# WestlyPark/StyleRenderer

Measured on AMD Instinct MI355X. Metric: generator fwd+bwd images/sec at 256^2, higher is better.
Workload: dtype f32

## Files before the change

### stylerenderer_amd/csrc/conv_wino.h

```cpp
#pragma once
#include <hip/hip_runtime.h>
#include <stdint.h>

struct WinoParams {
    const float* in;
    const float* u;
    const float* iscale;
    const float* oscale;
    const float* obias;
    float* out;
    int B, C, N, H, W;
    int tiles_x, tiles_y, tiles_n;
    int nba;
    const float* nz;
    const float* nz_w;
    const float* abias;
    int64_t nz_bstride;
    float alpha, gain;
    int ks, kchunks;
    float* partial;
};

struct WinoNba {
    const float* nz;
    const float* nz_w;
    const float* abias;
    int64_t nz_bstride;
    float alpha, gain;
};

bool sr_wino_eligible(int64_t B, int64_t C, int64_t N, int64_t H, int64_t W, const void* in, const void* out);
int64_t sr_wino_scratch_floats(int64_t C, int64_t N);
int sr_wino_split(int64_t B, int64_t C, int64_t N, int64_t H, int64_t W);
int64_t sr_wino_partial_floats(int64_t B, int64_t C, int64_t N, int64_t H, int64_t W);
int sr_wino_conv3x3(float* out, const float* in, const float* wt, int64_t ldw, const float* iscale,
                    const float* oscale, const float* obias, int64_t B, int64_t C, int64_t N, int64_t H, int64_t W,
                    float* u_scratch, hipStream_t st, const WinoNba* nba = nullptr, bool u_ready = false);

bool sr_wgrad_wino_eligible(int64_t B, int64_t C, int64_t N, int64_t H, int64_t W, const void* x, const void* gy);
int64_t sr_wgrad_wino_scratch_floats(int64_t B, int64_t C, int64_t N, int64_t H, int64_t W);
int sr_wgrad_wino_3x3(float* dwt, const float* x, const float* gy, const float* xscale, const float* gscale,
                      int64_t B, int64_t C, int64_t N, int64_t H, int64_t W, float* scratch, hipStream_t st);
```

### stylerenderer_amd/csrc/conv_wino.hip

```cpp
#include <type_traits>
#include "common.h"
#include "conv_wino.h"
#include <cstdlib>

namespace {

typedef float f32x16 __attribute__((ext_vector_type(16)));
typedef const void __attribute__((address_space(1)))* gptr_t;
typedef void __attribute__((address_space(3)))* lptr_t;

__device__ __attribute__((aligned(16))) const float g_wino_zero[4] = {0.f, 0.f, 0.f, 0.f};

constexpr int TW = 16, TH = 4;
constexpr int NB = 64;
constexpr int EH = 2 * TH + 2;
constexpr int LEAD = 3;
constexpr int EWP = 40;
constexpr int PLANE = EH * EWP;

#ifdef WINO_TIMING
__device__ long long g_wino_stamps[8 * 16384];
#define WINO_STAMP(i) do { if (tid == 0) { g_wino_stamps[(blockIdx.x & 16383) * 8 + (i)] = wall_clock64(); } } while (0)
#else
#define WINO_STAMP(i)
#endif

template <int KC>
struct WG {
    static constexpr int CQ = KC / 4;
    static constexpr int PPS = CQ * 512;
    static constexpr int UV = 8 * PPS;
    static constexpr int U_INSTR = UV / 256;
    static constexpr int D_FLOATS = KC * PLANE;
    static constexpr int D_INSTR = (D_FLOATS / 4 + 63) / 64;
    static constexpr int D_BUF = D_INSTR * 256;
    static constexpr int D_PER_WAVE = (D_INSTR + 3) / 4;
    static constexpr int PAD = 4 * UV + 2 * D_BUF;
    static constexpr int STY = PAD + 3 * 256;
};

template <int KC>
__global__ __launch_bounds__(256) void k_conv_wino(const WinoParams p) {
#if __HIP_DEVICE_COMPILE__
    using G = WG<KC>;
    extern __shared__ __attribute__((aligned(16))) float smem[];
    float* const ubuf = smem;
    float* const vbuf = smem + 2 * G::UV;
    float* const dbuf = smem + 4 * G::UV + 1;
    float* const sty = smem + G::STY;

    const int nwg = gridDim.x;
    int bid = blockIdx.x;
    {
        const int q = nwg / SR_NUM_XCD, r = nwg % SR_NUM_XCD, xcd = bid % SR_NUM_XCD;
        bid = (xcd < r ? xcd * (q + 1) : r * (q + 1) + (xcd - r) * q) + bid / SR_NUM_XCD;
    }
    const int slice = bid % p.ks;
    bid /= p.ks;
    const int n_t = bid % p.tiles_n;
    bid /= p.tiles_n;
    const int tx_i = bid % p.tiles_x;
    bid /= p.tiles_x;
    const int ty_i = bid % p.tiles_y;
    const int b = bid / p.tiles_y;
    const int oy0 = ty_i * (2 * TH), ox0 = tx_i * (2 * TW), n0 = n_t * NB;

    const int tid = threadIdx.x, lane = tid & 63;
    const int wave = __builtin_amdgcn_readfirstlane(tid >> 6);
    const int half = lane >> 5, l31 = lane & 31;
    const int wn = wave & 1, wt = wave >> 1;
    const int nchunks = p.kchunks;
    const int k_lo = slice * p.kchunks;
    const int all_chunks = p.C / KC;
    WINO_STAMP(0);
#ifdef WINO_TIMING
    const long long wino_c0 = clock64();
    if (tid == 0) {
        g_wino_stamps[(blockIdx.x & 16383) * 8 + 6] = __builtin_amdgcn_s_getreg((31 << 11) | 4);
        g_wino_stamps[(blockIdx.x & 16383) * 8 + 7] = __builtin_amdgcn_s_getreg((31 << 11) | 20);
    }
#endif

    int d_off[G::D_PER_WAVE];
#pragma unroll
    for (int i = 0; i < G::D_PER_WAVE; ++i) {
        const int j = wave + 4 * i;
        const int f = (j * 64 + lane) * 4;
        int off = 0x7FFFFFF0;
        if (j < G::D_INSTR && f < G::D_FLOATS) {
            const int c = f / PLANE, q = f % PLANE;
            const int r = q / EWP, cola = q % EWP;
            const int gy = oy0 - 1 + r, gx = ox0 - 4 + cola;
            if (gy >= 0 && gy < p.H && gx >= 0 && gx + 3 < p.W) off = ((c * p.H + gy) * p.W + gx) * 4;
        }
        d_off[i] = off;
    }
    const int chunk_in_bytes = KC * p.H * p.W * 4;
    const __amdgpu_buffer_rsrc_t r_in = __builtin_amdgcn_make_buffer_rsrc(
        const_cast<float*>(p.in + ((int64_t)b * p.C + (int64_t)k_lo * KC) * p.H * p.W), 0, nchunks * chunk_in_bytes,
        0x00020000);
    const __amdgpu_buffer_rsrc_t r_u = __builtin_amdgcn_make_buffer_rsrc(
        const_cast<float*>(p.u + ((int64_t)n_t * all_chunks + k_lo) * G::UV), 0, nchunks * G::UV * 4, 0x00020000);
    const int u_voff = lane * 16;

    auto dma_d1 = [&](int k, int buf, int i) {
        const int j = wave + 4 * i;
        float* dst = j < G::D_INSTR ? dbuf + buf * G::D_BUF + j * 256 : smem + G::PAD + (wave - 1) * 256;
        __builtin_amdgcn_raw_ptr_buffer_load_lds(r_in, (lptr_t)dst, 16, d_off[i], k * chunk_in_bytes, 0, 0);
    };
    auto dma_u1 = [&](int k, int buf, int i) {
        const int j = wave + 4 * i;
        __builtin_amdgcn_raw_ptr_buffer_load_lds(r_u, (lptr_t)(ubuf + buf * G::UV + j * 256), 16, u_voff,
                                                 (k * G::UV + j * 256) * 4, 0, 0);
    };
    auto dma_d = [&](int k, int buf) {
#pragma unroll
        for (int i = 0; i < G::D_PER_WAVE; ++i) dma_d1(k, buf, i);
    };
    auto dma_u = [&](int k, int buf) {
#pragma unroll
        for (int i = 0; i < G::U_INSTR / 4; ++i) dma_u1(k, buf, i);
    };

    static_assert(KC == 8, "two channel quads per chunk");
    const int t_cq = wave & 1, t_h = wave >> 1;
    const int t_ca = 4 * t_cq + t_h;
    const int t_rd = t_ca * PLANE + (2 * (lane >> 4)) * EWP + LEAD + 2 * (lane & 15);
    const int t_wr = t_cq * 512 + t_h * 128 + lane * 2;

    typedef float f2 __attribute__((ext_vector_type(2)));
    auto ld2 = [](const float* q) { return *reinterpret_cast<const f2*>(q); };
    auto st2 = [](float* q, f2 v) { *reinterpret_cast<f2*>(q) = v; };
    auto pk_add = [](f2 x, f2 y) { f2 r; asm("v_pk_add_f32 %0, %1, %2" : "=v"(r) : "v"(x), "v"(y)); return r; };
    auto pk_sub = [](f2 x, f2 y) {
        f2 r;
        asm("v_pk_add_f32 %0, %1, %2 neg_lo:[0,1] neg_hi:[0,1]" : "=v"(r) : "v"(x), "v"(y));
        return r;
    };
    auto pk_mul_s = [](f2 x, f2 sv, int ch) {
        f2 r;
        if (ch == 0) asm("v_pk_mul_f32 %0, %1, %2 op_sel:[0,0] op_sel_hi:[1,0]" : "=v"(r) : "v"(x), "v"(sv));
        else asm("v_pk_mul_f32 %0, %1, %2 op_sel:[0,1] op_sel_hi:[1,1]" : "=v"(r) : "v"(x), "v"(sv));
        return r;
    };
    auto pk_fms_s = [](f2 x, f2 sv, f2 y, int ch) {
        f2 r;
        if (ch == 0)
            asm("v_pk_fma_f32 %0, %1, %2, %3 op_sel:[0,0,0] op_sel_hi:[1,0,1] neg_lo:[0,0,1] neg_hi:[0,0,1]"
                : "=v"(r) : "v"(x), "v"(sv), "v"(y));
        else
            asm("v_pk_fma_f32 %0, %1, %2, %3 op_sel:[0,1,0] op_sel_hi:[1,1,1] neg_lo:[0,0,1] neg_hi:[0,0,1]"
                : "=v"(r) : "v"(x), "v"(sv), "v"(y));
        return r;
    };
    auto pk_fnma_s = [](f2 x, f2 sv, f2 y, int ch) {
        f2 r;
        if (ch == 0)
            asm("v_pk_fma_f32 %0, %1, %2, %3 op_sel:[0,0,0] op_sel_hi:[1,0,1] neg_lo:[1,0,0] neg_hi:[1,0,0]"
                : "=v"(r) : "v"(x), "v"(sv), "v"(y));
        else
            asm("v_pk_fma_f32 %0, %1, %2, %3 op_sel:[0,1,0] op_sel_hi:[1,1,1] neg_lo:[1,0,0] neg_hi:[1,0,0]"
                : "=v"(r) : "v"(x), "v"(sv), "v"(y));
        return r;
    };
    auto col01 = [](f2 tp, f2 tq) {
        f2 r;
        asm("v_pk_add_f32 %0, %1, %2 op_sel:[0,0] op_sel_hi:[1,0] neg_lo:[0,1] neg_hi:[0,0]" : "=v"(r) : "v"(tp), "v"(tq));
        return r;
    };
    auto col23 = [](f2 tp, f2 tq) {
        f2 r;
        asm("v_pk_add_f32 %0, %1, %2 op_sel:[0,1] op_sel_hi:[1,1] neg_lo:[0,1] neg_hi:[1,0]" : "=v"(r) : "v"(tq), "v"(tp));
        return r;
    };
    struct XF {
        f2 P[2][4], Q[2][4];
        f2 sp[2][2], sq[2][2];
        f2 tp[2][4], tq[2][4];
        f2 o01[2][4], o23[2][4];
    };
    auto xf_read = [&](XF& x, const float* d0, int r) {
#pragma unroll
        for (int ch = 0; ch < 2; ++ch) {
            x.P[ch][r] = ld2(d0 + ch * 2 * PLANE + r * EWP);
            x.Q[ch][r] = ld2(d0 + ch * 2 * PLANE + r * EWP + 2);
        }
    };
    auto xf_step = [&](XF& x, int step, f2 sv) {
#pragma unroll
        for (int ch = 0; ch < 2; ++ch) {
            if (step == 0) {
                x.sp[ch][0] = pk_mul_s(x.P[ch][1], sv, ch);
                x.sp[ch][1] = pk_mul_s(x.P[ch][2], sv, ch);
                x.sq[ch][0] = pk_mul_s(x.Q[ch][1], sv, ch);
                x.sq[ch][1] = pk_mul_s(x.Q[ch][2], sv, ch);
                x.tp[ch][0] = pk_fms_s(x.P[ch][0], sv, x.sp[ch][1], ch);
                x.tq[ch][0] = pk_fms_s(x.Q[ch][0], sv, x.sq[ch][1], ch);
            } else if (step == 1) {
                x.tp[ch][1] = pk_add(x.sp[ch][0], x.sp[ch][1]);
                x.tq[ch][1] = pk_add(x.sq[ch][0], x.sq[ch][1]);
                x.tp[ch][2] = pk_sub(x.sp[ch][1], x.sp[ch][0]);
                x.tq[ch][2] = pk_sub(x.sq[ch][1], x.sq[ch][0]);
                x.tp[ch][3] = pk_fnma_s(x.P[ch][3], sv, x.sp[ch][0], ch);
                x.tq[ch][3] = pk_fnma_s(x.Q[ch][3], sv, x.sq[ch][0], ch);
            } else {
#pragma unroll
                for (int q = 2 * (step - 2); q < 2 * (step - 2) + 2; ++q) {
                    x.o01[ch][q] = col01(x.tp[ch][q], x.tq[ch][q]);
                    x.o23[ch][q] = col23(x.tp[ch][q], x.tq[ch][q]);
                }
            }
        }
    };
    auto xf_write = [&](const XF& x, float* vout, int q) {
#pragma unroll
        for (int ch = 0; ch < 2; ++ch) {
            st2(vout + (2 * q) * G::PPS + ch * 256, x.o01[ch][q]);
            st2(vout + (2 * q + 1) * G::PPS + ch * 256, x.o23[ch][q]);
        }
    };
    auto transform = [&](int k, int dsel, int vsel) {
        const float* d0 = dbuf + dsel * G::D_BUF + t_rd;
        float* v = vbuf + vsel * G::UV + t_wr;
        f2 sv;
        sv.x = sty[k * KC + t_ca];
        sv.y = sty[k * KC + t_ca + 2];
        XF x;
#pragma unroll
        for (int r = 0; r < 4; ++r) xf_read(x, d0, r);
#pragma unroll
        for (int st = 0; st < 4; ++st) xf_step(x, st, sv);
#pragma unroll
        for (int q = 0; q < 4; ++q) xf_write(x, v, q);
    };

    f32x16 acc[16];
#pragma unroll
    for (int pos = 0; pos < 16; ++pos)
#pragma unroll
        for (int r = 0; r < 16; ++r) acc[pos][r] = 0.0f;

    const int a_off = (half * 64 + wn * 32 + l31) * 2;
    const int b_off = (half * 64 + wt * 32 + l31) * 2;

    dma_d(0, 0);
    dma_u(0, 0);
    if (nchunks > 1) dma_d(1, 1);
    for (int c = tid; c < nchunks * KC; c += 256)
        sty[c] = p.iscale ? p.iscale[(int64_t)b * p.C + k_lo * KC + c] : 1.0f;
    __builtin_amdgcn_s_waitcnt(0x0F70);
    __syncthreads();
    WINO_STAMP(1);
    transform(0, 0, 0);
    WINO_STAMP(2);

    static_assert(KC == 8, "the slot schedule below is written for two channel quads per chunk");
    f2 au[2][2][8], bv[2][2][8];
    auto mfma_step = [&](int cq, int m) {
        const int e = m >> 4, pos = m & 15, pp = pos >> 1;
        if (pos & 1) acc[pos] = __builtin_amdgcn_mfma_f32_32x32x2f32(au[cq][e][pp].y, bv[cq][e][pp].y, acc[pos], 0, 0, 0);
        else acc[pos] = __builtin_amdgcn_mfma_f32_32x32x2f32(au[cq][e][pp].x, bv[cq][e][pp].x, acc[pos], 0, 0, 0);
    };
    auto body = [&](int k, auto first_tag) {
        constexpr bool FIRST = decltype(first_tag)::value;
        __builtin_amdgcn_s_waitcnt(0x0F70);
        __syncthreads();
        const int kd = min(k + 2, nchunks - 1), ku = min(k + 1, nchunks - 1);
        const float* ub = ubuf + (k & 1) * G::UV + a_off;
        const float* vb_ = vbuf + (k & 1) * G::UV + b_off;
        const int kn = (k + 1 < nchunks) ? k + 1 : k;
        const float* d0 = dbuf + ((k + 1) & 1) * G::D_BUF + t_rd;
        float* vout = vbuf + ((k + 1) & 1) * G::UV + t_wr;
        f2 sab;
        sab.x = sty[kn * KC + t_ca];
        sab.y = sty[kn * KC + t_ca + 2];
        XF x;
        auto load_ops = [&](int cq, int pp) {
#pragma unroll
            for (int e = 0; e < 2; ++e) {
                au[cq][e][pp] = ld2(ub + pp * G::PPS + cq * 512 + e * 256);
                bv[cq][e][pp] = ld2(vb_ + pp * G::PPS + cq * 512 + e * 256);
            }
        };
#ifndef WINO_RD
#define WINO_RD "0123"
#define WINO_ST "4567"
#define WINO_WR "CDEF"
#define WINO_L0 "4567"
#define WINO_L1 "89AB"
#define WINO_DD "45"
#define WINO_DU "89AB"
#endif
        constexpr char RD[] = WINO_RD, ST[] = WINO_ST, WR[] = WINO_WR, L0[] = WINO_L0, L1[] = WINO_L1, DD[] = WINO_DD,
                       DU[] = WINO_DU;
        static_assert(sizeof(RD) == 5 && sizeof(ST) == 5 && sizeof(WR) == 5 && sizeof(L0) == 5 && sizeof(L1) == 5 &&
                      sizeof(DD) == 3 && sizeof(DU) == 5, "schedule strings");
        static_assert(G::D_PER_WAVE == 4 && G::U_INSTR / 4 == 8, "4 halo + 8 weight DMA instructions per wave");
#pragma unroll
        for (int s = 0; s < 16; ++s) {
            const int cq = (s < 8) ? 1 : 0, j = s & 7;
            const char d = s < 10 ? '0' + s : 'A' + (s - 10);
            if (!(FIRST && s < 8)) {
#pragma unroll
                for (int u = 0; u < 4; ++u) mfma_step(cq, 4 * j + u);
            }
#pragma unroll
            for (int i = 0; i < 4; ++i) {
                if (L0[i] == d) { load_ops(0, 2 * i); load_ops(0, 2 * i + 1); }
                if (L1[i] == d) { load_ops(1, 2 * i); load_ops(1, 2 * i + 1); }
            }
#ifndef WINO_NO_DMA
#pragma unroll
            for (int i = 0; i < 4; ++i) {
                if (i < 2 && DD[i] == d) { dma_d1(kd, k & 1, 2 * i); dma_d1(kd, k & 1, 2 * i + 1); }
                if (DU[i] == d) { dma_u1(ku, (k + 1) & 1, 2 * i); dma_u1(ku, (k + 1) & 1, 2 * i + 1); }
            }
#endif
#ifndef WINO_NO_XFORM
#pragma unroll
            for (int i = 0; i < 4; ++i) if (RD[i] == d) xf_read(x, d0, i);
#pragma unroll
            for (int i = 0; i < 4; ++i) if (ST[i] == d) xf_step(x, i, sab);
#pragma unroll
            for (int i = 0; i < 4; ++i) if (WR[i] == d) xf_write(x, vout, i);
#endif
            __builtin_amdgcn_sched_barrier(0);
        }
    };
    body(0, std::true_type{});
    for (int k = 1; k < nchunks; ++k) body(k, std::false_type{});
#pragma unroll
    for (int m = 0; m < 32; ++m) mfma_step(1, m);

    __builtin_amdgcn_s_waitcnt(0x0F70);
    WINO_STAMP(3);

    const int tile = wt * 32 + l31;
    const int oy = oy0 + 2 * (tile >> 4), ox = ox0 + 2 * (tile & 15);
    const int64_t plane = (int64_t)p.H * p.W;
    float nzv[2][2] = {{0.0f, 0.0f}, {0.0f, 0.0f}};
    if (p.nba && p.nz) {
#pragma clang fp contract(off)
        const float nw = p.nz_w[0];
        const float* nzp = p.nz + b * p.nz_bstride + (int64_t)oy * p.W + ox;
#pragma unroll
        for (int a = 0; a < 2; ++a) {
            nzv[a][0] = nw * nzp[a * p.W];
            nzv[a][1] = nw * nzp[a * p.W + 1];
        }
    }
#pragma unroll
    for (int r = 0; r < 16; ++r) {
        const int n = n0 + wn * 32 + (r & 3) + 8 * (r >> 2) + 4 * half;
        float s[2][4];
#pragma unroll
        for (int j = 0; j < 4; ++j) {
            const float m0 = acc[j][r], m1 = acc[4 + j][r], m2 = acc[8 + j][r], m3 = acc[12 + j][r];
            s[0][j] = (m0 + m1) + m2;
            s[1][j] = (m1 - m2) - m3;
        }
        if (p.ks > 1) {
            float* o = p.partial + (((int64_t)slice * p.B + b) * p.N + n) * plane + (int64_t)oy * p.W + ox;
            *reinterpret_cast<float2*>(o) = make_float2((s[0][0] + s[0][1]) + s[0][2], (s[0][1] - s[0][2]) - s[0][3]);
            *reinterpret_cast<float2*>(o + p.W) = make_float2((s[1][0] + s[1][1]) + s[1][2], (s[1][1] - s[1][2]) - s[1][3]);
            continue;
        }
        const float os = p.oscale ? p.oscale[(int64_t)b * p.N + n] : 1.0f;
        const float ob = p.obias ? p.obias[n] : 0.0f;
        float* o = p.out + ((int64_t)b * p.N + n) * plane + (int64_t)oy * p.W + ox;
        const float ab = (p.nba && p.abias) ? p.abias[n] : 0.0f;
        float y[2][2];
#pragma unroll
        for (int a = 0; a < 2; ++a) {
            const float y0 = (s[a][0] + s[a][1]) + s[a][2];
            const float y1 = (s[a][1] - s[a][2]) - s[a][3];
            float v0 = y0 * os + ob, v1 = y1 * os + ob;
            if (p.nba) {
#pragma clang fp contract(off)
                v0 = v0 + nzv[a][0];
                v1 = v1 + nzv[a][1];
                v0 = v0 + ab;
                v1 = v1 + ab;
                v0 = ((v0 > 0.0f) ? v0 : v0 * p.alpha) * p.gain;
                v1 = ((v1 > 0.0f) ? v1 : v1 * p.alpha) * p.gain;
            }
            y[a][0] = v0;
            y[a][1] = v1;
        }
        *reinterpret_cast<float2*>(o) = make_float2(y[0][0], y[0][1]);
        *reinterpret_cast<float2*>(o + p.W) = make_float2(y[1][0], y[1][1]);
    }
    WINO_STAMP(4);
#ifdef WINO_TIMING
    if (tid == 0) g_wino_stamps[(blockIdx.x & 16383) * 8 + 5] = clock64() - wino_c0;
#endif
#endif
}

__global__ __launch_bounds__(256) void k_wino_reduce(const WinoParams p) {
    const int64_t plane = (int64_t)p.H * p.W, total4 = (int64_t)p.B * p.N * plane / 4;
    const int64_t slab4 = total4;
    for (int64_t i = (int64_t)blockIdx.x * 256 + threadIdx.x; i < total4; i += (int64_t)gridDim.x * 256) {
        const float4* src = reinterpret_cast<const float4*>(p.partial) + i;
        float4 a = src[0];
        for (int s = 1; s < p.ks; ++s) {
            const float4 q = src[s * slab4];
            a.x += q.x; a.y += q.y; a.z += q.z; a.w += q.w;
        }
        const int64_t row = (i * 4) / plane;
        const int n = (int)(row % p.N), b = (int)(row / p.N);
        const int64_t pix = i * 4 - row * plane;
        const float os = p.oscale ? p.oscale[row] : 1.0f;
        const float ob = p.obias ? p.obias[n] : 0.0f;
        float v[4] = {a.x * os + ob, a.y * os + ob, a.z * os + ob, a.w * os + ob};
        if (p.nba) {
#pragma clang fp contract(off)
            const float ab = p.abias ? p.abias[n] : 0.0f;
            float nz[4] = {0.0f, 0.0f, 0.0f, 0.0f};
            if (p.nz) {
                const float nw = p.nz_w[0];
                const float4 q = *reinterpret_cast<const float4*>(p.nz + b * p.nz_bstride + pix);
                nz[0] = nw * q.x; nz[1] = nw * q.y; nz[2] = nw * q.z; nz[3] = nw * q.w;
            }
#pragma unroll
            for (int j = 0; j < 4; ++j) {
                float t = v[j] + nz[j];
                t = t + ab;
                v[j] = ((t > 0.0f) ? t : t * p.alpha) * p.gain;
            }
        }
        reinterpret_cast<float4*>(p.out)[i] = make_float4(v[0], v[1], v[2], v[3]);
    }
}

template <int KC>
__global__ __launch_bounds__(64) void k_wino_weights(float* __restrict__ u, const float* __restrict__ wt, int C,
                                                     int N, int ldw) {
    using G = WG<KC>;
    const int n = blockIdx.x * 64 + threadIdx.x, c = blockIdx.y;
    float g[3][3];
#pragma unroll
    for (int t = 0; t < 9; ++t) g[t / 3][t % 3] = wt[((int64_t)t * C + c) * ldw + n];
    float h[4][3];
#pragma unroll
    for (int j = 0; j < 3; ++j) {
        h[0][j] = g[0][j];
        h[1][j] = 0.5f * ((g[0][j] + g[2][j]) + g[1][j]);
        h[2][j] = 0.5f * ((g[0][j] + g[2][j]) - g[1][j]);
        h[3][j] = g[2][j];
    }
    const int cl = c % KC, cq = cl / 4, e = (cl % 4) / 2, hh = cl % 2;
    float* dst = u + ((int64_t)blockIdx.x * (C / KC) + c / KC) * G::UV + cq * 512 + e * 256 + hh * 128 + threadIdx.x * 2;
#pragma unroll
    for (int i = 0; i < 4; ++i) {
        *reinterpret_cast<float2*>(dst + (2 * i) * G::PPS) = make_float2(h[i][0], 0.5f * ((h[i][0] + h[i][2]) + h[i][1]));
        *reinterpret_cast<float2*>(dst + (2 * i + 1) * G::PPS) = make_float2(0.5f * ((h[i][0] + h[i][2]) - h[i][1]), h[i][2]);
    }
}

template <int KC>
int launch(const WinoParams& p, float* u, const float* wt, int ldw, hipStream_t st, bool u_ready) {
    using G = WG<KC>;
    const int lds = (G::STY + p.kchunks * KC) * 4;
    auto kern = k_conv_wino<KC>;
    static bool configured = false;
    if (!configured) {
        if (hipFuncSetAttribute(reinterpret_cast<const void*>(kern), hipFuncAttributeMaxDynamicSharedMemorySize,
                                160 * 1024) != hipSuccess) {
            (void)hipGetLastError();
            return SR_EINVAL;
        }
        configured = true;
    }
    if (!u_ready) hipLaunchKernelGGL(k_wino_weights<KC>, dim3(p.N / 64, p.C), dim3(64), 0, st, u, wt, p.C, p.N, ldw);
    const int64_t blocks = (int64_t)p.tiles_n * p.tiles_x * p.tiles_y * p.B * p.ks;
    hipLaunchKernelGGL(kern, dim3((unsigned)blocks), dim3(256), lds, st, p);
    if (p.ks > 1) {
        const int64_t total4 = (int64_t)p.B * p.N * p.H * p.W / 4;
        int64_t grid = (total4 + 255) / 256;
        if (grid > 8192) grid = 8192;
        hipLaunchKernelGGL(k_wino_reduce, dim3((unsigned)grid), dim3(256), 0, st, p);
    }
    return sr_launch_status();
}

}

#ifdef WINO_TIMING
extern "C" int sr_debug_wino_stamps(long long* host, int n) {
    return (int)hipMemcpyFromSymbol(host, HIP_SYMBOL(g_wino_stamps), (size_t)n * sizeof(long long));
}
#endif

bool sr_wino_eligible(int64_t B, int64_t C, int64_t N, int64_t H, int64_t W, const void* in, const void* out) {
    if (B <= 0 || C % 8 != 0 || N % 64 != 0 || H % 8 != 0 || W % 32 != 0) return false;
    if (C > 512 || B * ((W / 32) * (H / 8)) * (N / 64) > 0x7FFFFFFFLL) return false;
    if (C * H * W >= (1LL << 29) - 4 || 16 * C * 64 >= (1LL << 29)) return false;
    return ((reinterpret_cast<uintptr_t>(in) | reinterpret_cast<uintptr_t>(out)) & 15) == 0;
}

int64_t sr_wino_scratch_floats(int64_t C, int64_t N) { return 16 * C * N; }

int sr_wino_split(int64_t B, int64_t C, int64_t N, int64_t H, int64_t W) {
    const char* e = std::getenv("SR_WINO_SPLIT");
    if (e && e[0] == '0') return 1;
    const int64_t blocks = B * (W / (2 * TW)) * (H / (2 * TH)) * (N / NB), nchunks = C / 8;
    int ks = 1;
    while (blocks * ks < 192 && ks < 8 && nchunks % (2 * ks) == 0 && nchunks / (2 * ks) >= 8) ks *= 2;
    return ks;
}
int64_t sr_wino_partial_floats(int64_t B, int64_t C, int64_t N, int64_t H, int64_t W) {
    const int ks = sr_wino_split(B, C, N, H, W);
    return ks > 1 ? (int64_t)ks * B * N * H * W : 0;
}

int sr_wino_conv3x3(float* out, const float* in, const float* wt, int64_t ldw, const float* iscale,
                    const float* oscale, const float* obias, int64_t B, int64_t C, int64_t N, int64_t H, int64_t W,
                    float* u_scratch, hipStream_t st, const WinoNba* nba, bool u_ready) {
    WinoParams p;
    p.in = in; p.u = u_scratch; p.iscale = iscale; p.oscale = oscale; p.obias = obias; p.out = out;
    p.nba = nba ? 1 : 0;
    p.nz = nba ? nba->nz : nullptr; p.nz_w = nba ? nba->nz_w : nullptr; p.abias = nba ? nba->abias : nullptr;
    p.nz_bstride = nba ? nba->nz_bstride : 0; p.alpha = nba ? nba->alpha : 0.0f; p.gain = nba ? nba->gain : 1.0f;
    p.B = (int)B; p.C = (int)C; p.N = (int)N; p.H = (int)H; p.W = (int)W;
    p.tiles_x = (int)(W / (2 * TW)); p.tiles_y = (int)(H / (2 * TH)); p.tiles_n = (int)(N / NB);
    p.ks = sr_wino_split(B, C, N, H, W);
    p.kchunks = (int)(C / 8) / p.ks;
    p.partial = u_scratch + sr_wino_scratch_floats(C, N);
    return launch<8>(p, u_scratch, wt, (int)ldw, st, u_ready);
}
```

Baseline: 549.1.

## Make Winograd conv kernel persistent, overlapping next tile prologue with epilogue

Turns the Winograd 3x3 conv kernel into a persistent kernel: the grid is capped at the CU count and each workgroup loops over virtual tile IDs. Before running the current tile's epilogue it decodes the next tile, computes its DMA offsets, loads its style scales and issues the first halo/weight DMAs, so the next tile's loads overlap the output stores. The accumulator zeroing moves into the first MFMA step. Epilogue per-channel scales are loaded once per lane and broadcast with readlane. Risks include higher register pressure, worse load balance when tile counts are not a multiple of the grid, and buffer-parity bookkeeping across tiles.

```diff
diff --git a/stylerenderer_amd/csrc/conv_wino.h b/stylerenderer_amd/csrc/conv_wino.h
--- a/stylerenderer_amd/csrc/conv_wino.h
+++ b/stylerenderer_amd/csrc/conv_wino.h
@@ -19,6 +19,7 @@
     float alpha, gain;
     int ks, kchunks;
     float* partial;
+    int total;
 };
 
 struct WinoNba {
@@ -33,6 +34,7 @@
 int64_t sr_wino_scratch_floats(int64_t C, int64_t N);
 int sr_wino_split(int64_t B, int64_t C, int64_t N, int64_t H, int64_t W);
 int64_t sr_wino_partial_floats(int64_t B, int64_t C, int64_t N, int64_t H, int64_t W);
+int sr_wino_grid(int64_t tiles);
 int sr_wino_conv3x3(float* out, const float* in, const float* wt, int64_t ldw, const float* iscale,
                     const float* oscale, const float* obias, int64_t B, int64_t C, int64_t N, int64_t H, int64_t W,
                     float* u_scratch, hipStream_t st, const WinoNba* nba = nullptr, bool u_ready = false);
diff --git a/stylerenderer_amd/csrc/conv_wino.hip b/stylerenderer_amd/csrc/conv_wino.hip
--- a/stylerenderer_amd/csrc/conv_wino.hip
+++ b/stylerenderer_amd/csrc/conv_wino.hip
@@ -20,9 +20,11 @@
 
 #ifdef WINO_TIMING
 __device__ long long g_wino_stamps[8 * 16384];
-#define WINO_STAMP(i) do { if (tid == 0) { g_wino_stamps[(blockIdx.x & 16383) * 8 + (i)] = wall_clock64(); } } while (0)
+#define WINO_STAMP(i) do { if (tid == 0) { g_wino_stamps[(v & 16383) * 8 + (i)] = wall_clock64(); } } while (0)
+#define WINO_CLOCK() do { if (tid == 0) g_wino_stamps[(v & 16383) * 8 + 5] = clock64() - wino_c0; } while (0)
 #else
 #define WINO_STAMP(i)
+#define WINO_CLOCK()
 #endif
 
 template <int KC>
@@ -49,58 +51,53 @@
     float* const dbuf = smem + 4 * G::UV + 1;
     float* const sty = smem + G::STY;
 
-    const int nwg = gridDim.x;
-    int bid = blockIdx.x;
-    {
-        const int q = nwg / SR_NUM_XCD, r = nwg % SR_NUM_XCD, xcd = bid % SR_NUM_XCD;
-        bid = (xcd < r ? xcd * (q + 1) : r * (q + 1) + (xcd - r) * q) + bid / SR_NUM_XCD;
-    }
-    const int slice = bid % p.ks;
-    bid /= p.ks;
-    const int n_t = bid % p.tiles_n;
-    bid /= p.tiles_n;
-    const int tx_i = bid % p.tiles_x;
-    bid /= p.tiles_x;
-    const int ty_i = bid % p.tiles_y;
-    const int b = bid / p.tiles_y;
-    const int oy0 = ty_i * (2 * TH), ox0 = tx_i * (2 * TW), n0 = n_t * NB;
-
     const int tid = threadIdx.x, lane = tid & 63;
     const int wave = __builtin_amdgcn_readfirstlane(tid >> 6);
     const int half = lane >> 5, l31 = lane & 31;
     const int wn = wave & 1, wt = wave >> 1;
     const int nchunks = p.kchunks;
-    const int k_lo = slice * p.kchunks;
     const int all_chunks = p.C / KC;
-    WINO_STAMP(0);
-#ifdef WINO_TIMING
-    const long long wino_c0 = clock64();
-    if (tid == 0) {
-        g_wino_stamps[(blockIdx.x & 16383) * 8 + 6] = __builtin_amdgcn_s_getreg((31 << 11) | 4);
-        g_wino_stamps[(blockIdx.x & 16383) * 8 + 7] = __builtin_amdgcn_s_getreg((31 << 11) | 20);
-    }
-#endif
+    const int chunk_in_bytes = KC * p.H * p.W * 4;
+
+    struct Tile { int b, slice, n_t, oy0, ox0; };
+    const int xq = p.total / SR_NUM_XCD, xr = p.total % SR_NUM_XCD;
+    auto decode = [&](int vid) {
+        const int xcd = vid % SR_NUM_XCD;
+        int bid = (xcd < xr ? xcd * (xq + 1) : xr * (xq + 1) + (xcd - xr) * xq) + vid / SR_NUM_XCD;
+        Tile t;
+        t.slice = bid % p.ks;
+        bid /= p.ks;
+        t.n_t = bid % p.tiles_n;
+        bid /= p.tiles_n;
+        t.ox0 = (bid % p.tiles_x) * (2 * TW);
+        bid /= p.tiles_x;
+        t.oy0 = (bid % p.tiles_y) * (2 * TH);
+        t.b = bid / p.tiles_y;
+        return t;
+    };
 
     int d_off[G::D_PER_WAVE];
-#pragma unroll
-    for (int i = 0; i < G::D_PER_WAVE; ++i) {
-        const int j = wave + 4 * i;
-        const int f = (j * 64 + lane) * 4;
-        int off = 0x7FFFFFF0;
-        if (j < G::D_INSTR && f < G::D_FLOATS) {
+    __amdgpu_buffer_rsrc_t r_in, r_u;
+    auto aim = [&](const Tile& t) {
+        int ln = lane;
+        asm volatile("" : "+v"(ln));
+#pragma unroll
+        for (int i = 0; i < G::D_PER_WAVE; ++i) {
+            const int j = wave + 4 * i;
+            const int f = (j * 64 + ln) * 4;
             const int c = f / PLANE, q = f % PLANE;
             const int r = q / EWP, cola = q % EWP;
-            const int gy = oy0 - 1 + r, gx = ox0 - 4 + cola;
-            if (gy >= 0 && gy < p.H && gx >= 0 && gx + 3 < p.W) off = ((c * p.H + gy) * p.W + gx) * 4;
-        }
-        d_off[i] = off;
-    }
-    const int chunk_in_bytes = KC * p.H * p.W * 4;
-    const __amdgpu_buffer_rsrc_t r_in = __builtin_amdgcn_make_buffer_rsrc(
-        const_cast<float*>(p.in + ((int64_t)b * p.C + (int64_t)k_lo * KC) * p.H * p.W), 0, nchunks * chunk_in_bytes,
-        0x00020000);
-    const __amdgpu_buffer_rsrc_t r_u = __builtin_amdgcn_make_buffer_rsrc(
-        const_cast<float*>(p.u + ((int64_t)n_t * all_chunks + k_lo) * G::UV), 0, nchunks * G::UV * 4, 0x00020000);
+            const int gy = t.oy0 - 1 + r, gx = t.ox0 - 4 + cola;
+            const bool ok = (j < G::D_INSTR) & (f < G::D_FLOATS) & (gy >= 0) & (gy < p.H) & (gx >= 0) & (gx + 3 < p.W);
+            d_off[i] = ok ? ((c * p.H + gy) * p.W + gx) * 4 : 0x7FFFFFF0;
+        }
+        const int k_lo = t.slice * nchunks;
+        r_in = __builtin_amdgcn_make_buffer_rsrc(
+            const_cast<float*>(p.in + ((int64_t)t.b * p.C + (int64_t)k_lo * KC) * p.H * p.W), 0,
+            nchunks * chunk_in_bytes, 0x00020000);
+        r_u = __builtin_amdgcn_make_buffer_rsrc(
+            const_cast<float*>(p.u + ((int64_t)t.n_t * all_chunks + k_lo) * G::UV), 0, nchunks * G::UV * 4, 0x00020000);
+    };
     const int u_voff = lane * 16;
 
     auto dma_d1 = [&](int k, int buf, int i) {
@@ -235,53 +232,80 @@
     };
 
     f32x16 acc[16];
-#pragma unroll
-    for (int pos = 0; pos < 16; ++pos)
-#pragma unroll
-        for (int r = 0; r < 16; ++r) acc[pos][r] = 0.0f;
 
     const int a_off = (half * 64 + wn * 32 + l31) * 2;
     const int b_off = (half * 64 + wt * 32 + l31) * 2;
 
-    dma_d(0, 0);
-    dma_u(0, 0);
-    if (nchunks > 1) dma_d(1, 1);
-    for (int c = tid; c < nchunks * KC; c += 256)
-        sty[c] = p.iscale ? p.iscale[(int64_t)b * p.C + k_lo * KC + c] : 1.0f;
-    __builtin_amdgcn_s_waitcnt(0x0F70);
-    __syncthreads();
-    WINO_STAMP(1);
-    transform(0, 0, 0);
-    WINO_STAMP(2);
-
-    static_assert(KC == 8, "the slot schedule below is written for two channel quads per chunk");
-    f2 au[2][2][8], bv[2][2][8];
-    auto mfma_step = [&](int cq, int m) {
-        const int e = m >> 4, pos = m & 15, pp = pos >> 1;
-        if (pos & 1) acc[pos] = __builtin_amdgcn_mfma_f32_32x32x2f32(au[cq][e][pp].y, bv[cq][e][pp].y, acc[pos], 0, 0, 0);
-        else acc[pos] = __builtin_amdgcn_mfma_f32_32x32x2f32(au[cq][e][pp].x, bv[cq][e][pp].x, acc[pos], 0, 0, 0);
-    };
-    auto body = [&](int k, auto first_tag) {
-        constexpr bool FIRST = decltype(first_tag)::value;
-        __builtin_amdgcn_s_waitcnt(0x0F70);
-        __syncthreads();
-        const int kd = min(k + 2, nchunks - 1), ku = min(k + 1, nchunks - 1);
-        const float* ub = ubuf + (k & 1) * G::UV + a_off;
-        const float* vb_ = vbuf + (k & 1) * G::UV + b_off;
-        const int kn = (k + 1 < nchunks) ? k + 1 : k;
-        const float* d0 = dbuf + ((k + 1) & 1) * G::D_BUF + t_rd;
-        float* vout = vbuf + ((k + 1) & 1) * G::UV + t_wr;
-        f2 sab;
-        sab.x = sty[kn * KC + t_ca];
-        sab.y = sty[kn * KC + t_ca + 2];
-        XF x;
-        auto load_ops = [&](int cq, int pp) {
-#pragma unroll
-            for (int e = 0; e < 2; ++e) {
-                au[cq][e][pp] = ld2(ub + pp * G::PPS + cq * 512 + e * 256);
-                bv[cq][e][pp] = ld2(vb_ + pp * G::PPS + cq * 512 + e * 256);
-            }
+    static_assert(KC == 8, "style row: at most 512 channels per tile, see sr_wino_eligible");
+    float sreg[2];
+    auto style_load = [&](const Tile& t) {
+        int th = tid;
+        asm volatile("" : "+v"(th));
+#pragma unroll
+        for (int i = 0; i < 2; ++i) {
+            const int c = th + 256 * i;
+            sreg[i] = (p.iscale && c < nchunks * KC) ? p.iscale[(int64_t)t.b * p.C + t.slice * nchunks * KC + c] : 1.0f;
+        }
+    };
+    auto style_store = [&]() {
+        int th = tid;
+        asm volatile("" : "+v"(th));
+#pragma unroll
+        for (int i = 0; i < 2; ++i) {
+            const int c = th + 256 * i;
+            if (c < nchunks * KC) sty[c] = sreg[i];
+        }
+    };
+    auto issue_first = [&](int par) {
+        dma_d(0, par);
+        dma_u(0, par);
+        dma_d(min(1, nchunks - 1), par ^ 1);
+    };
+
+    int v = blockIdx.x, par = 0;
+    Tile cur = decode(v);
+#ifdef WINO_TIMING
+    const int wino_hw0 = __builtin_amdgcn_s_getreg((31 << 11) | 4), wino_hw1 = __builtin_amdgcn_s_getreg((31 << 11) | 20);
+#endif
+    aim(cur);
+    style_load(cur);
+    issue_first(0);
+    for (;;) {
+        static_assert(KC == 8, "the slot schedule below is written for two channel quads per chunk");
+        f2 au[2][2][8], bv[2][2][8];
+        auto mfma_step = [&](int cq, int m, bool start) {
+            const int e = m >> 4, pos = m & 15, pp = pos >> 1;
+            f32x16 c;
+            if (start) {
+#pragma unroll
+                for (int r = 0; r < 16; ++r) c[r] = 0.0f;
+            } else {
+                c = acc[pos];
+            }
+            if (pos & 1) acc[pos] = __builtin_amdgcn_mfma_f32_32x32x2f32(au[cq][e][pp].y, bv[cq][e][pp].y, c, 0, 0, 0);
+            else acc[pos] = __builtin_amdgcn_mfma_f32_32x32x2f32(au[cq][e][pp].x, bv[cq][e][pp].x, c, 0, 0, 0);
         };
+        auto body = [&](int k, int kb, auto first_tag) {
+            constexpr bool FIRST = decltype(first_tag)::value;
+            __builtin_amdgcn_s_waitcnt(0x0F70);
+            __syncthreads();
+            const int kd = min(k + 2, nchunks - 1), ku = min(k + 1, nchunks - 1);
+            const float* ub = ubuf + (kb & 1) * G::UV + a_off;
+            const float* vb_ = vbuf + (kb & 1) * G::UV + b_off;
+            const int kn = (k + 1 < nchunks) ? k + 1 : k;
+            const float* d0 = dbuf + ((kb + 1) & 1) * G::D_BUF + t_rd;
+            float* vout = vbuf + ((kb + 1) & 1) * G::UV + t_wr;
+            f2 sab;
+            sab.x = sty[kn * KC + t_ca];
+            sab.y = sty[kn * KC + t_ca + 2];
+            XF x;
+            auto load_ops = [&](int cq, int pp) {
+#pragma unroll
+                for (int e = 0; e < 2; ++e) {
+                    au[cq][e][pp] = ld2(ub + pp * G::PPS + cq * 512 + e * 256);
+                    bv[cq][e][pp] = ld2(vb_ + pp * G::PPS + cq * 512 + e * 256);
+                }
+            };
 #ifndef WINO_RD
 #define WINO_RD "0123"
 #define WINO_ST "4567"
@@ -291,109 +315,165 @@
 #define WINO_DD "45"
 #define WINO_DU "89AB"
 #endif
-        constexpr char RD[] = WINO_RD, ST[] = WINO_ST, WR[] = WINO_WR, L0[] = WINO_L0, L1[] = WINO_L1, DD[] = WINO_DD,
-                       DU[] = WINO_DU;
-        static_assert(sizeof(RD) == 5 && sizeof(ST) == 5 && sizeof(WR) == 5 && sizeof(L0) == 5 && sizeof(L1) == 5 &&
-                      sizeof(DD) == 3 && sizeof(DU) == 5, "schedule strings");
-        static_assert(G::D_PER_WAVE == 4 && G::U_INSTR / 4 == 8, "4 halo + 8 weight DMA instructions per wave");
-#pragma unroll
-        for (int s = 0; s < 16; ++s) {
-            const int cq = (s < 8) ? 1 : 0, j = s & 7;
-            const char d = s < 10 ? '0' + s : 'A' + (s - 10);
-            if (!(FIRST && s < 8)) {
-#pragma unroll
-                for (int u = 0; u < 4; ++u) mfma_step(cq, 4 * j + u);
-            }
-#pragma unroll
-            for (int i = 0; i < 4; ++i) {
-                if (L0[i] == d) { load_ops(0, 2 * i); load_ops(0, 2 * i + 1); }
-                if (L1[i] == d) { load_ops(1, 2 * i); load_ops(1, 2 * i + 1); }
-            }
+            constexpr char RD[] = WINO_RD, ST[] = WINO_ST, WR[] = WINO_WR, L0[] = WINO_L0, L1[] = WINO_L1, DD[] = WINO_DD,
+                           DU[] = WINO_DU;
+            static_assert(sizeof(RD) == 5 && sizeof(ST) == 5 && sizeof(WR) == 5 && sizeof(L0) == 5 && sizeof(L1) == 5 &&
+                          sizeof(DD) == 3 && sizeof(DU) == 5, "schedule strings");
+            static_assert(G::D_PER_WAVE == 4 && G::U_INSTR / 4 == 8, "4 halo + 8 weight DMA instructions per wave");
+#pragma unroll
+            for (int s = 0; s < 16; ++s) {
+                const int cq = (s < 8) ? 1 : 0, j = s & 7;
+                const char d = s < 10 ? '0' + s : 'A' + (s - 10);
+                if (!(FIRST && s < 8)) {
+#pragma unroll
+                    for (int u = 0; u < 4; ++u) mfma_step(cq, 4 * j + u, FIRST && 4 * j + u < 16);
+                }
+#pragma unroll
+                for (int i = 0; i < 4; ++i) {
+                    if (L0[i] == d) { load_ops(0, 2 * i); load_ops(0, 2 * i + 1); }
+                    if (L1[i] == d) { load_ops(1, 2 * i); load_ops(1, 2 * i + 1); }
+                }
 #ifndef WINO_NO_DMA
 #pragma unroll
-            for (int i = 0; i < 4; ++i) {
-                if (i < 2 && DD[i] == d) { dma_d1(kd, k & 1, 2 * i); dma_d1(kd, k & 1, 2 * i + 1); }
-                if (DU[i] == d) { dma_u1(ku, (k + 1) & 1, 2 * i); dma_u1(ku, (k + 1) & 1, 2 * i + 1); }
-            }
+                for (int i = 0; i < 4; ++i) {
+                    if (i < 2 && DD[i] == d) { dma_d1(kd, kb & 1, 2 * i); dma_d1(kd, kb & 1, 2 * i + 1); }
+                    if (DU[i] == d) { dma_u1(ku, (kb + 1) & 1, 2 * i); dma_u1(ku, (kb + 1) & 1, 2 * i + 1); }
+                }
 #endif
 #ifndef WINO_NO_XFORM
 #pragma unroll
-            for (int i = 0; i < 4; ++i) if (RD[i] == d) xf_read(x, d0, i);
-#pragma unroll
-            for (int i = 0; i < 4; ++i) if (ST[i] == d) xf_step(x, i, sab);
-#pragma unroll
-            for (int i = 0; i < 4; ++i) if (WR[i] == d) xf_write(x, vout, i);
-#endif
-            __builtin_amdgcn_sched_barrier(0);
-        }
-    };
-    body(0, std::true_type{});
-    for (int k = 1; k < nchunks; ++k) body(k, std::false_type{});
-#pragma unroll
-    for (int m = 0; m < 32; ++m) mfma_step(1, m);
-
+                for (int i = 0; i < 4; ++i) if (RD[i] == d) xf_read(x, d0, i);
+#pragma unroll
+                for (int i = 0; i < 4; ++i) if (ST[i] == d) xf_step(x, i, sab);
+#pragma unroll
+                for (int i = 0; i < 4; ++i) if (WR[i] == d) xf_write(x, vout, i);
+#endif
+                __builtin_amdgcn_sched_barrier(0);
+            }
+        };
+        WINO_STAMP(0);
+#ifdef WINO_TIMING
+        const long long wino_c0 = clock64();
+        if (tid == 0) {
+            g_wino_stamps[(v & 16383) * 8 + 6] = wino_hw0;
+            g_wino_stamps[(v & 16383) * 8 + 7] = wino_hw1;
+        }
+#endif
+        style_store();
+        __builtin_amdgcn_s_waitcnt(0x0F70);
+        __syncthreads();
+        WINO_STAMP(1);
+        transform(0, par, par);
+        WINO_STAMP(2);
+        body(0, par, std::true_type{});
+        for (int k = 1; k < nchunks; ++k) body(k, k + par, std::false_type{});
+        WINO_STAMP(3);
+
+        const int b = cur.b, n0 = cur.n_t * NB;
+        const int tile = wt * 32 + l31;
+        const int oy = cur.oy0 + 2 * (tile >> 4), ox = cur.ox0 + 2 * (tile & 15);
+        const int64_t plane = (int64_t)p.H * p.W;
+        const int nl = n0 + wn * 32 + 4 * half;
+        float e_os = 1.0f, e_ob = 0.0f, e_ab = 0.0f;
+        float nzv[2][2] = {{0.0f, 0.0f}, {0.0f, 0.0f}}, nzw = 0.0f;
+        if (p.ks == 1) {
+            const int nc = n0 + wn * 32 + l31;
+            if (p.oscale) e_os = p.oscale[(int64_t)b * p.N + nc];
+            if (p.obias) e_ob = p.obias[nc];
+            if (p.nba && p.abias) e_ab = p.abias[nc];
+            if (p.nba && p.nz) {
+                nzw = p.nz_w[0];
+                const float* nzp = p.nz + b * p.nz_bstride + (int64_t)oy * p.W + ox;
+#pragma unroll
+                for (int a = 0; a < 2; ++a) {
+                    nzv[a][0] = nzp[a * p.W];
+                    nzv[a][1] = nzp[a * p.W + 1];
+                }
+            }
+        }
+        __builtin_amdgcn_sched_barrier(0);
+#pragma unroll
+        for (int m = 0; m < 32; ++m) mfma_step(1, m, false);
+        __builtin_amdgcn_sched_barrier(0);
+
+        auto epilogue = [&]() {
+            if (p.nba && p.nz) {
+#pragma clang fp contract(off)
+#pragma unroll
+                for (int a = 0; a < 2; ++a) {
+                    nzv[a][0] = nzw * nzv[a][0];
+                    nzv[a][1] = nzw * nzv[a][1];
+                }
+            }
+#pragma unroll
+            for (int r = 0; r < 16; ++r) {
+                const int n = nl + (r & 3) + 8 * (r >> 2);
+                float s[2][4];
+#pragma unroll
+                for (int j = 0; j < 4; ++j) {
+                    const float m0 = acc[j][r], m1 = acc[4 + j][r], m2 = acc[8 + j][r], m3 = acc[12 + j][r];
+                    s[0][j] = (m0 + m1) + m2;
+                    s[1][j] = (m1 - m2) - m3;
+                }
+                if (p.ks > 1) {
+                    float* o = p.partial + (((int64_t)cur.slice * p.B + b) * p.N + n) * plane + (int64_t)oy * p.W + ox;
+                    *reinterpret_cast<float2*>(o) = make_float2((s[0][0] + s[0][1]) + s[0][2], (s[0][1] - s[0][2]) - s[0][3]);
+                    *reinterpret_cast<float2*>(o + p.W) = make_float2((s[1][0] + s[1][1]) + s[1][2], (s[1][1] - s[1][2]) - s[1][3]);
+                    continue;
+                }
+                const int c0 = (r & 3) + 8 * (r >> 2);
+                auto row = [&](float held) {
+                    const int bits = __float_as_int(held);
+                    const int lo = __builtin_amdgcn_readlane(bits, c0), hi = __builtin_amdgcn_readlane(bits, c0 + 4);
+                    return __int_as_float(half ? hi : lo);
+                };
+                const float os = row(e_os);
+                const float ob = row(e_ob);
+                float* o = p.out + ((int64_t)b * p.N + n) * plane + (int64_t)oy * p.W + ox;
+                const float ab = row(e_ab);
+                float y[2][2];
+#pragma unroll
+                for (int a = 0; a < 2; ++a) {
+                    const float y0 = (s[a][0] + s[a][1]) + s[a][2];
+                    const float y1 = (s[a][1] - s[a][2]) - s[a][3];
+                    float v0 = y0 * os + ob, v1 = y1 * os + ob;
+                    if (p.nba) {
+#pragma clang fp contract(off)
+                        v0 = v0 + nzv[a][0];
+                        v1 = v1 + nzv[a][1];
+                        v0 = v0 + ab;
+                        v1 = v1 + ab;
+                        v0 = ((v0 > 0.0f) ? v0 : v0 * p.alpha) * p.gain;
+                        v1 = ((v1 > 0.0f) ? v1 : v1 * p.alpha) * p.gain;
+                    }
+                    y[a][0] = v0;
+                    y[a][1] = v1;
+                }
+                *reinterpret_cast<float2*>(o) = make_float2(y[0][0], y[0][1]);
+                *reinterpret_cast<float2*>(o + p.W) = make_float2(y[1][0], y[1][1]);
+            }
+        };
+
+        const int vn = v + (int)gridDim.x;
+        if (vn >= p.total) {
+            epilogue();
+            WINO_STAMP(4);
+            WINO_CLOCK();
+            break;
+        }
+        const Tile nxt = decode(vn);
+        aim(nxt);
+        par = (par + nchunks) & 1;
+        style_load(nxt);
+        issue_first(par);
+        __builtin_amdgcn_sched_barrier(0);
+        epilogue();
+        WINO_STAMP(4);
+        WINO_CLOCK();
+        cur = nxt;
+        v = vn;
+    }
     __builtin_amdgcn_s_waitcnt(0x0F70);
-    WINO_STAMP(3);
-
-    const int tile = wt * 32 + l31;
-    const int oy = oy0 + 2 * (tile >> 4), ox = ox0 + 2 * (tile & 15);
-    const int64_t plane = (int64_t)p.H * p.W;
-    float nzv[2][2] = {{0.0f, 0.0f}, {0.0f, 0.0f}};
-    if (p.nba && p.nz) {
-#pragma clang fp contract(off)
-        const float nw = p.nz_w[0];
-        const float* nzp = p.nz + b * p.nz_bstride + (int64_t)oy * p.W + ox;
-#pragma unroll
-        for (int a = 0; a < 2; ++a) {
-            nzv[a][0] = nw * nzp[a * p.W];
-            nzv[a][1] = nw * nzp[a * p.W + 1];
-        }
-    }
-#pragma unroll
-    for (int r = 0; r < 16; ++r) {
-        const int n = n0 + wn * 32 + (r & 3) + 8 * (r >> 2) + 4 * half;
-        float s[2][4];
-#pragma unroll
-        for (int j = 0; j < 4; ++j) {
-            const float m0 = acc[j][r], m1 = acc[4 + j][r], m2 = acc[8 + j][r], m3 = acc[12 + j][r];
-            s[0][j] = (m0 + m1) + m2;
-            s[1][j] = (m1 - m2) - m3;
-        }
-        if (p.ks > 1) {
-            float* o = p.partial + (((int64_t)slice * p.B + b) * p.N + n) * plane + (int64_t)oy * p.W + ox;
-            *reinterpret_cast<float2*>(o) = make_float2((s[0][0] + s[0][1]) + s[0][2], (s[0][1] - s[0][2]) - s[0][3]);
-            *reinterpret_cast<float2*>(o + p.W) = make_float2((s[1][0] + s[1][1]) + s[1][2], (s[1][1] - s[1][2]) - s[1][3]);
-            continue;
-        }
-        const float os = p.oscale ? p.oscale[(int64_t)b * p.N + n] : 1.0f;
-        const float ob = p.obias ? p.obias[n] : 0.0f;
-        float* o = p.out + ((int64_t)b * p.N + n) * plane + (int64_t)oy * p.W + ox;
-        const float ab = (p.nba && p.abias) ? p.abias[n] : 0.0f;
-        float y[2][2];
-#pragma unroll
-        for (int a = 0; a < 2; ++a) {
-            const float y0 = (s[a][0] + s[a][1]) + s[a][2];
-            const float y1 = (s[a][1] - s[a][2]) - s[a][3];
-            float v0 = y0 * os + ob, v1 = y1 * os + ob;
-            if (p.nba) {
-#pragma clang fp contract(off)
-                v0 = v0 + nzv[a][0];
-                v1 = v1 + nzv[a][1];
-                v0 = v0 + ab;
-                v1 = v1 + ab;
-                v0 = ((v0 > 0.0f) ? v0 : v0 * p.alpha) * p.gain;
-                v1 = ((v1 > 0.0f) ? v1 : v1 * p.alpha) * p.gain;
-            }
-            y[a][0] = v0;
-            y[a][1] = v1;
-        }
-        *reinterpret_cast<float2*>(o) = make_float2(y[0][0], y[0][1]);
-        *reinterpret_cast<float2*>(o + p.W) = make_float2(y[1][0], y[1][1]);
-    }
-    WINO_STAMP(4);
-#ifdef WINO_TIMING
-    if (tid == 0) g_wino_stamps[(blockIdx.x & 16383) * 8 + 5] = clock64() - wino_c0;
-#endif
 #endif
 }
 
@@ -473,8 +553,7 @@
         configured = true;
     }
     if (!u_ready) hipLaunchKernelGGL(k_wino_weights<KC>, dim3(p.N / 64, p.C), dim3(64), 0, st, u, wt, p.C, p.N, ldw);
-    const int64_t blocks = (int64_t)p.tiles_n * p.tiles_x * p.tiles_y * p.B * p.ks;
-    hipLaunchKernelGGL(kern, dim3((unsigned)blocks), dim3(256), lds, st, p);
+    hipLaunchKernelGGL(kern, dim3((unsigned)sr_wino_grid(p.total)), dim3(256), lds, st, p);
     if (p.ks > 1) {
         const int64_t total4 = (int64_t)p.B * p.N * p.H * p.W / 4;
         int64_t grid = (total4 + 255) / 256;
@@ -508,6 +587,17 @@
     int ks = 1;
     while (blocks * ks < 192 && ks < 8 && nchunks % (2 * ks) == 0 && nchunks / (2 * ks) >= 8) ks *= 2;
     return ks;
+}
+int sr_wino_grid(int64_t tiles) {
+    const char* e = std::getenv("SR_WINO_PERSIST");
+    int64_t g = tiles;
+    if (!(e && e[0] == '0') && g > SR_NUM_CU) g = SR_NUM_CU;
+    const char* c = std::getenv("SR_WINO_MAX_WG");
+    if (c && c[0]) {
+        const long cap = std::strtol(c, nullptr, 10);
+        if (cap >= 1 && cap < g) g = cap;
+    }
+    return (int)g;
 }
 int64_t sr_wino_partial_floats(int64_t B, int64_t C, int64_t N, int64_t H, int64_t W) {
     const int ks = sr_wino_split(B, C, N, H, W);
@@ -527,5 +617,6 @@
     p.ks = sr_wino_split(B, C, N, H, W);
     p.kchunks = (int)(C / 8) / p.ks;
     p.partial = u_scratch + sr_wino_scratch_floats(C, N);
+    p.total = p.tiles_n * p.tiles_x * p.tiles_y * p.B * p.ks;
     return launch<8>(p, u_scratch, wt, (int)ldw, st, u_ready);
 }
```

Result: no change. 550.2 (median of 5 runs) (+0.2%).
